# decadenza/SimpleStereo

Measured on AMD Instinct MI355X. Metric: disparity MPixels/s (H*W*nDisp per second), higher is better.
Workload: dtype f32

## Files before the change

### simplestereo_amd/build.py

```python
import os
import shutil
import subprocess

_PKG = os.path.dirname(os.path.abspath(__file__))
_SRC = os.path.join(_PKG, "csrc")
LIB_PATH = os.path.join(_PKG, "libssamd.so")
HIPCC_FLAGS = ["--offload-arch=gfx950", "-O3", "-std=c++17", "-shared", "-fPIC", "-fno-slp-vectorize",
               "-Wno-int-to-pointer-cast"]


def _sources():
    return sorted(os.path.join(_SRC, f) for f in os.listdir(_SRC) if f.endswith((".hip", ".h", ".inc")))


def needs_build():
    if not os.path.exists(LIB_PATH):
        return True
    t = os.path.getmtime(LIB_PATH)
    deps = _sources() + [os.path.join(os.path.dirname(_PKG), "include", "ssamd.h")]
    return any(os.path.getmtime(s) > t for s in deps if os.path.exists(s))


UNITS = [("ssamd_api.hip", []),
         ("asw_pipe_tu.hip", ["-mllvm", "--amdgpu-sched-strategy=max-memory-clause"]),
         ("asw_wave6_tu.hip", ["-mllvm", "--amdgpu-sched-strategy=max-ilp"])]


def build_native(force=False, verbose=False):
    if not force and not needs_build():
        return LIB_PATH
    hipcc = shutil.which("hipcc") or "/opt/rocm/bin/hipcc"
    if not os.path.exists(hipcc):
        raise RuntimeError("hipcc not found: libssamd.so cannot be built (ROCm toolchain required)")
    flags = [f for f in HIPCC_FLAGS if f != "-shared"]
    objs, procs = [], []
    for src, extra in UNITS:
        obj = os.path.join(_SRC, os.path.splitext(src)[0] + ".o")
        cmd = [hipcc] + flags + extra + ["-c", "-o", obj, os.path.join(_SRC, src)]
        if verbose:
            print(" ".join(cmd))
        procs.append((cmd, subprocess.Popen(cmd)))
        objs.append(obj)
    for cmd, p in procs:
        if p.wait() != 0:
            raise subprocess.CalledProcessError(p.returncode, cmd)
    cmd = [hipcc, "--offload-arch=gfx950", "-shared", "-fPIC", "-o", LIB_PATH + ".tmp"] + objs
    if verbose:
        print(" ".join(cmd))
    subprocess.check_call(cmd)
    os.replace(LIB_PATH + ".tmp", LIB_PATH)
    for o in objs:
        os.remove(o)
    return LIB_PATH


if __name__ == "__main__":
    print(build_native(force=True, verbose=True))
```

### simplestereo_amd/csrc/asw_kernels.hip.h

```cpp
#pragma once
#include "common.hip.h"

namespace ssamd {

static constexpr int ASW_RX = 8;
static constexpr int ASW_RD = 4;
static constexpr int ASW_WB = 4;
static constexpr int ASW_MAX_THREADS = 768;
__host__ __device__ constexpr int asw_nwr(int rx) { return (rx + ASW_RD - 1 + 3) / 4 * 4; }
static_assert(ASW_RD == 4 && asw_nwr(8) == 12 && asw_nwr(4) == 8, "the main loop is unrolled for 8x4 and 4x4 register tiles");

struct AswGeom {
    int Tx, XG, DG, Dc, nchunks, threads;
    int Rx;
    int nL, nR, nRc, SR, Se, emask;
    int SL, hL, hR;
    int wseg, wlen;
    int JC;
    int e2;
    int e_bytes;
    int pipe;
    int NC, JCmax;
    int dephase;
    int wave_rx;
    int off_wL, off_wR, off_e, off_labL, off_labR, off_bgrL, off_bgrR, off_bestL, off_bestR, off_cen, off_prox;
    int lds_bytes;
    int lds_bytes_evol;
};

struct AswExactQueue {
    u64 *entries;
    uint32_t *ekeys;
    unsigned int *counter;
    unsigned char *flagL, *flagR;
    unsigned char *zeroL, *zeroR;
    unsigned char *zrow;
    unsigned int W;
    unsigned int cap;
    uint32_t tol;
    float sat_abs;
    uint32_t deep;
};

struct AswArgs {
    const PixRec *recL, *recR;
    const float *prox;
    u64 *keyL;
    u64 *keyR;
    int16_t *disp;
    const unsigned char *evol;
    int erow0, erows, evolW;
    float *costs;
    int cost_keys;
    int H, W, win, pad, minD, maxD, row0, rows;
    int ystep;
    int yb0;
    int yskip_at, yskip;
    float kC;
    AswExactQueue xq;
    AswGeom g;
};

struct AswPipeTileId { int win, XG, DG, JC; };
__host__ __device__ constexpr int asw_cx_round_up(int v, int m) { return (v + m - 1) / m * m; }
__host__ __device__ constexpr int asw_cx_max(int a, int b) { return a > b ? a : b; }
__host__ __device__ constexpr AswGeom asw_pipe_geom_constexpr(AswPipeTileId t)
{
    AswGeom g{};
    const int win = t.win, p = win / 2;
    g.Rx = 8; g.JC = t.JC; g.pipe = 1; g.wave_rx = 0; g.e2 = 1; g.nchunks = 1;
    g.NC = (win + t.JC / 2) / t.JC;
    g.JCmax = asw_cx_max(t.JC, win - (g.NC - 1) * t.JC);
    g.XG = t.XG; g.DG = t.DG;
    g.Tx = 8 * t.XG; g.Dc = ASW_RD * t.DG;
    g.threads = asw_cx_round_up(t.XG * t.DG, 64);
    g.dephase = g.threads / 64 >= 12 ? 1 : 0;
    g.nL = g.Tx + 2 * p;
    g.nRc = g.Tx + g.Dc - 1;
    g.nR = g.nRc + 2 * p;
    g.hL = 0; g.hR = 0;
    g.SL = asw_cx_round_up(g.Tx, 4);
    g.SR = asw_cx_round_up(g.nRc + 1, 4);
    g.Se = 16 * ((t.DG + 3) / 4);
    g.emask = 0;
    const int wrows = 2 * g.JCmax;
    int off = 0;
    g.off_wL = off; off = (off + wrows * g.SL * 4 + 15) & ~15;
    g.off_wR = off; off = (off + wrows * g.SR * 4 + 15) & ~15;
    g.e_bytes = (g.nL * g.Se + 15) & ~15;
    g.off_e = off; off = (off + g.e_bytes * 2 + 15) & ~15;
    g.off_labL = off; off = (off + g.nL * 16 * 2 + 15) & ~15;
    g.off_labR = off; off = (off + g.nR * 16 * 2 + 15) & ~15;
    g.off_bestL = off; off = (off + g.Tx * 8 + 15) & ~15;
    g.off_bestR = off; off = (off + (g.nRc + 1) * 8 + 15) & ~15;
    g.off_cen = off; off = (off + (g.Tx + g.nRc) * 16 + 15) & ~15;
    g.off_prox = off; off = (off + win * 4 * 2 + 15) & ~15;
    g.lds_bytes_evol = off;
    g.off_bgrL = off; off = (off + g.nL * 4 * 2 + 15) & ~15;
    g.off_bgrR = off; off = (off + g.nR * 4 * 2 + 15) & ~15;
    g.lds_bytes = off;
    return g;
}
template <int SLC, int SRC, int SEC> struct AswPipeTile { static constexpr AswPipeTileId id{35, 1, 1, 16}; };
template <> struct AswPipeTile<120, 316, 208> { static constexpr AswPipeTileId id{35, 15, 49, 16}; };
template <> struct AswPipeTile<88, 348, 272> { static constexpr AswPipeTileId id{35, 11, 65, 16}; };
template <> struct AswPipeTile<216, 284, 80> { static constexpr AswPipeTileId id{35, 27, 17, 16}; };
inline bool asw_pipe_geom_matches(const AswGeom &a, const AswGeom &b)
{
    return a.pipe == b.pipe && a.Rx == b.Rx && a.JC == b.JC && a.NC == b.NC && a.JCmax == b.JCmax && a.XG == b.XG && a.DG == b.DG && a.Tx == b.Tx &&
           a.Dc == b.Dc && a.threads == b.threads && a.dephase == b.dephase && a.nL == b.nL && a.nRc == b.nRc && a.nR == b.nR && a.SL == b.SL &&
           a.SR == b.SR && a.Se == b.Se && a.e_bytes == b.e_bytes && a.off_wL == b.off_wL && a.off_wR == b.off_wR && a.off_e == b.off_e &&
           a.off_labL == b.off_labL && a.off_labR == b.off_labR && a.off_bestL == b.off_bestL && a.off_bestR == b.off_bestR &&
           a.off_cen == b.off_cen && a.off_prox == b.off_prox && a.off_bgrL == b.off_bgrL && a.off_bgrR == b.off_bgrR &&
           a.lds_bytes == b.lds_bytes && a.lds_bytes_evol == b.lds_bytes_evol && a.e2 == b.e2;
// ... 574 lines not shown
```

### simplestereo_amd/csrc/asw_pipe_kernel.hip.h

```cpp
#pragma once
#include "asw_kernels.hip.h"
#ifndef SSAMD_KERNEL_TU
#include "lab_kernels.hip.h"
#endif

namespace ssamd {

#ifndef SSAMD_KERNEL_TU
static constexpr int TADV_COLS = 64;
template <bool BYTES>
__device__ __forceinline__ void asw_tad_tile(const void *__restrict__ srcL, const void *__restrict__ srcR, unsigned char *__restrict__ evol,
                                             int W, int pad, int minD, int Dc, int Se, int erow0, int erows, int evolW, int rd, long long npix_total,
                                             int bx, int by, int bz, char *smem)
{
    uint32_t *const sL = reinterpret_cast<uint32_t *>(smem);
    uint32_t *const sR = sL + TADV_COLS;
    const int r = erow0 + by, z = bz, uc0 = bx * TADV_COLS;
    const int P = Se >> 2, dlo = minD + z * Dc, dhi = dlo + Dc - 1;
    const int u0 = uc0 - pad, xr0 = u0 - dhi;
    auto pixel = [&](const void *src, int col) -> uint32_t {
        const size_t q = (size_t)r * W + col;
        if constexpr (BYTES) {
            typedef uint32_t __attribute__((aligned(1))) u32_unaligned;
            const uint8_t *const b = reinterpret_cast<const uint8_t *>(src) + 3 * q;
// ... 41 lines not shown
    }
}

__global__ __launch_bounds__(256) void asw_tad_volume_kernel(const PixRec *__restrict__ recL, const PixRec *__restrict__ recR,
                                                             unsigned char *__restrict__ evol, int W, int pad, int minD, int Dc,
                                                             int Se, int erow0, int erows, int evolW, int rd = 4)
{
    extern __shared__ __attribute__((aligned(16))) char smem[];
    asw_tad_tile<false>(recL, recR, evol, W, pad, minD, Dc, Se, erow0, erows, evolW, rd, 0, blockIdx.x, blockIdx.y, blockIdx.z, smem);
}

struct AswPrepassArgs {
    const uint8_t *bgrL, *bgrR;
    PixRec *recL, *recR;
    unsigned char *evol;
    long long npix_total;
    int W, pad, minD, Dc, Se, erow0, erows, evolW, rd;
    int lab_blocks, ex, ey;
};
__global__ __launch_bounds__(256) void asw_prepass_kernel(const AswPrepassArgs P)
{
    extern __shared__ __attribute__((aligned(16))) char smem[];
    if ((int)blockIdx.x < P.lab_blocks) {
        SSAMD_LAB_TABLES_IN_LDS(T)
        const long long np = (long long)P.erows * P.W, first = (long long)P.erow0 * P.W;
        const uint8_t *const bl = P.bgrL + 3 * first, *const br = P.bgrR + 3 * first;
        PixRec *const rl = P.recL + first, *const rr = P.recR + first;
        typedef uint32_t __attribute__((aligned(1))) u32_unaligned;
        for (long long q = (long long)blockIdx.x * blockDim.x + threadIdx.x; q < 2 * np; q += (long long)P.lab_blocks * blockDim.x) {
            const bool right = q >= np;
            const long long p = right ? q - np : q;
            const uint8_t *const bgr = right ? br : bl;
            uint32_t B, G, R;
            if (p + 1 < np) {
                const uint32_t v = *reinterpret_cast<const u32_unaligned *>(bgr + 3 * p);
                B = v & 0xff; G = (v >> 8) & 0xff; R = (v >> 16) & 0xff;
            } else {
                B = bgr[3 * p]; G = bgr[3 * p + 1]; R = bgr[3 * p + 2];
            }
            PixRec o;
            bgr_to_lab(B, G, R, o.L, o.a, o.b, T);
            o.bgrx = B | (G << 8) | (R << 16);
            (right ? rr : rl)[p] = o;
        }
        return;
    }
    const int b = (int)blockIdx.x - P.lab_blocks, bx = b % P.ex, by = (b / P.ex) % P.ey, bz = b / (P.ex * P.ey);
    asw_tad_tile<true>(P.bgrL, P.bgrR, P.evol, P.W, P.pad, P.minD, P.Dc, P.Se, P.erow0, P.erows, P.evolW, P.rd, P.npix_total, bx, by, bz, smem);
}

#endif

template <bool WITH_COSTS, int SLC = 0, int SRC = 0, int SEC = 0, bool CG = false>
__global__ __launch_bounds__(ASW_MAX_THREADS, 3) void asw_aggregate_pipe_kernel(const AswArgs A)
{
    constexpr bool STATIC = SLC > 0;
    static_assert(!CG || STATIC, "compile-time geometry belongs to a static tile");
    constexpr int RX = ASW_RX;
    constexpr int NWR = asw_nwr(RX);
    extern __shared__ __attribute__((aligned(16))) char smem[];
    constexpr AswGeom SG = asw_pipe_geom_constexpr(AswPipeTile<SLC, SRC, SEC>::id);
    static_assert(!STATIC || (SG.SL == SLC && SG.SR == SRC && SG.Se == SEC), "the strides name the tile");
    const AswGeom &g = CG ? SG : A.g;
    float *const wL = reinterpret_cast<float *>(smem + g.off_wL);
    float *const wR = reinterpret_cast<float *>(smem + g.off_wR);
    unsigned char *const eT0 = reinterpret_cast<unsigned char *>(smem + g.off_e);
    float4 *const labL = reinterpret_cast<float4 *>(smem + g.off_labL);
    float4 *const labR = reinterpret_cast<float4 *>(smem + g.off_labR);
    uint32_t *const bgrL = reinterpret_cast<uint32_t *>(smem + g.off_bgrL);
    uint32_t *const bgrR = reinterpret_cast<uint32_t *>(smem + g.off_bgrR);
    u64 *const bestL = reinterpret_cast<u64 *>(smem + g.off_bestL);
    u64 *const bestR = reinterpret_cast<u64 *>(smem + g.off_bestR);
    float4 *const cenLab = reinterpret_cast<float4 *>(smem + g.off_cen);

    const int tid = threadIdx.x, nthr = blockDim.x;
    const int W = A.W, win = CG ? AswPipeTile<SLC, SRC, SEC>::id.win : A.win, p = CG ? AswPipeTile<SLC, SRC, SEC>::id.win / 2 : A.pad;
    const int Tx = g.Tx, Dc = g.Dc, nL = g.nL, nR = g.nR, nRc = g.nRc, SR = g.SR, Se = g.Se;
    const int JC = g.JC, NC = g.NC;
    int bx = blockIdx.x;
    if ((gridDim.x & 7) == 0) bx = (bx & 7) * (gridDim.x >> 3) + (bx >> 3);
    const int x0 = bx * Tx;
    const int y = asw_out_row(A, blockIdx.y);
    const int dlo = A.minD + blockIdx.z * Dc;
    const int dhi = dlo + Dc - 1;
    if (min(x0 + Tx - 1, W - 1) - dlo < 0) {
        if (A.disp)
            for (int k = threadIdx.x; k < Tx && x0 + k < W; k += blockDim.x)
                A.disp[(size_t)(y - A.row0) * W + x0 + k] = (int16_t)(x0 + k);
        return;
    }
    const int segL_lo = x0 - p, xrc_lo = x0 - dhi, segR_lo = xrc_lo - p;
    const int phase = g.dephase ? __builtin_amdgcn_readfirstlane((int)(threadIdx.x >> 8)) : 1;

    float accN[RX][ASW_RD], accS[RX][ASW_RD];
#pragma unroll
    for (int a = 0; a < RX; ++a)
#pragma unroll
        for (int b = 0; b < ASW_RD; ++b) { accN[a][b] = 0.f; accS[a][b] = 0.f; }

    for (int k = tid; k < Tx; k += nthr) bestL[k] = KEY_NONE;
    for (int k = tid; k <= nRc; k += nthr) bestR[k] = KEY_NONE;
    for (int c = tid; c < Tx + nRc; c += nthr) {
        const bool isL = c < Tx;
        const int ccol = isL ? x0 + c : xrc_lo + (c - Tx);
        float4 v = make_float4(0.f, 0.f, 0.f, 0.f);
        if ((unsigned)ccol < (unsigned)W) {
            const PixRec q = (isL ? A.recL : A.recR)[(size_t)y * W + ccol];
            v = make_float4(q.L, q.a, q.b, 1.f);
        }
        cenLab[c] = v;
    }

    const int i_lo = max(0, p - y), i_hi = min(win, A.H + p - y);

    auto stage_row = [&](int i) {
        int tids = threadIdx.x;
        asm volatile("" : "+v"(tids));
        const int buf = i & 1, r = y - p + i;
        const PixRec *const rowL = A.recL + (size_t)r * W;
        const PixRec *const rowR = A.recR + (size_t)r * W;
        for (int k = tids; k < nL + nR; k += nthr) {
            const bool isL = k < nL;
            const int idx = isL ? k : k - nL;
            const int col = (isL ? segL_lo : segR_lo) + idx;
            PixRec v;
            v.L = __builtin_inff();
            v.a = v.b = 0.f;
            v.bgrx = 0u;
            if ((unsigned)col < (unsigned)W) v = (isL ? rowL : rowR)[col];
            (isL ? labL + buf * nL : labR + buf * nR)[idx] = make_float4(v.L, v.a, v.b, 0.f);
            if (!A.evol) (isL ? bgrL + buf * nL : bgrR + buf * nR)[idx] = v.bgrx;
        }
    };
    auto build_e = [&](int i, int t_lo, int t_hi) {
        int tidb = threadIdx.x;
        asm volatile("" : "+v"(tidb));
        unsigned char *const eT = eT0 + (i & 1) * g.e_bytes;
        const uint32_t *const bgrLc = bgrL + (i & 1) * nL, *const bgrRc = bgrR + (i & 1) * nR;
        const int e_q = nthr / nL, e_r = nthr - e_q * nL;
        int t = t_lo + tidb;
        int sp = t / nL, ul = t - sp * nL;
        while (t < t_hi) {
            const uint32_t lp = bgrLc[ul];
            const uint32_t *const rp = bgrRc + (ul + (Dc - 1) - 8 * sp);
            uint32_t lo = 0, hi = 0;
#pragma unroll
            for (int k = 0; k < 4; ++k) {
                lo |= min(__builtin_amdgcn_sad_u8(lp, rp[-k], 0u), 40u) << (8 * k);
                hi |= min(__builtin_amdgcn_sad_u8(lp, rp[-4 - k], 0u), 40u) << (8 * k);
            }
            uint32_t *const dst = reinterpret_cast<uint32_t *>(eT + ul * Se) + 2 * sp;
            dst[0] = lo;
            if (2 * sp + 1 < g.DG) dst[1] = hi;
            t += nthr; ul += e_r; sp += e_q;
            if (ul >= nL) { ul -= nL; ++sp; }
        }
    };
    auto load_e = [&](int i) {
        int tidd = threadIdx.x;
        asm volatile("" : "+v"(tidd));
        const int r = y - p + i;
        const unsigned char *const src = A.evol + (((size_t)blockIdx.z * A.erows + (r - A.erow0)) * (size_t)A.evolW + x0) * Se;
        unsigned char *const dst = eT0 + (i & 1) * g.e_bytes;
        const int bytes = nL * Se, lane16 = (tidd & 63) * 16;
        for (int k = __builtin_amdgcn_readfirstlane(tidd >> 6) * 1024; k < bytes; k += (nthr >> 6) * 1024)
            if (k + lane16 < bytes)
                __builtin_amdgcn_global_load_lds((const void *)(src + k + lane16),
                                                 (__attribute__((address_space(3))) void *)(dst + k), 16, 0, 0);
    };
    auto build_weights = [&](int i, int jb, int je, int rb) {
        static_assert(ASW_WB == 4, "the remainder below is written out for batches of four");
        typedef const __attribute__((address_space(4))) float cfloat;
        int tidw = threadIdx.x;
        asm volatile("" : "+v"(tidw));
        const int wave = __builtin_amdgcn_readfirstlane(tidw >> 6), lane = tidw & 63;
        constexpr int NTHR = STATIC ? asw_cx_round_up((SLC / ASW_RX) * ((SRC - SLC) / ASW_RD), 64) : 0;
        static_assert(!STATIC || (SG.Tx == SLC && SG.nRc == SRC - 1 && SG.threads == NTHR), "the strides name the centres and the threads");
        const int TxB = STATIC ? SLC : Tx, nRcB = STATIC ? SRC - 1 : nRc, nw = (STATIC ? NTHR : nthr) >> 6;
        const int nLw = (TxB + 63) >> 6, ncw = nLw + ((nRcB + 63) >> 6);
        const float4 *const labLc = labL + (i & 1) * nL, *const labRc = labR + (i & 1) * nR;
        cfloat *const prow = reinterpret_cast<cfloat *>(reinterpret_cast<uintptr_t>(A.prox)) + i * win;
        auto batch = [&](auto n_, const float4 &cen, const float4 *sp, cfloat *pp, float *wp, int stride) {
            constexpr int N = decltype(n_)::value;
            float4 tp[N];
            float pr[N], wv[N];
#pragma unroll
            for (int u = 0; u < N; ++u) { tp[u] = sp[u]; pr[u] = pp[u]; }
#pragma unroll
            for (int u = 0; u < N; ++u) {
                asm volatile("" ::"v"(tp[u].w));
                const float dL = tp[u].x - cen.x, da = tp[u].y - cen.y, db = tp[u].z - cen.z;
                wv[u] = fmaf(db, db, fmaf(da, da, dL * dL));
            }
#pragma unroll
            for (int u = 0; u < N; ++u) wv[u] = __builtin_amdgcn_sqrtf(wv[u]);
#pragma unroll
            for (int u = 0; u < N; ++u) wv[u] = asw_weight_finish(wv[u], A.kC, pr[u]);
#pragma unroll
            for (int u = 0; u < N; ++u) wp[u * stride] = wv[u];
        };
        auto build_side = [&](auto left_, int cc, int jb_t, int je_t) {
            constexpr bool LEFT = decltype(left_)::value;
            const int stride = LEFT ? (STATIC ? SLC : g.SL) : (STATIC ? SRC : SR);
            if (cc >= (LEFT ? TxB : nRcB)) return;
            const float4 cen = cenLab[(LEFT ? 0 : TxB) + cc];
            asm volatile("" ::"v"(cen.w));
            const float4 *sp = (LEFT ? labLc : labRc) + cc + jb_t;
            cfloat *pp = prow + jb_t;
            float *wp = (LEFT ? wL : wR) + cc + (rb + jb_t - jb) * stride;
            int j = jb_t;
#pragma nounroll
            for (; j + ASW_WB <= je_t; j += ASW_WB, sp += ASW_WB, pp += ASW_WB, wp += ASW_WB * stride)
                batch(std::integral_constant<int, ASW_WB>{}, cen, sp, pp, wp, stride);
            const int rem = je_t - j;
            if (rem == 1) batch(std::integral_constant<int, 1>{}, cen, sp, pp, wp, stride);
            else if (rem == 2) batch(std::integral_constant<int, 2>{}, cen, sp, pp, wp, stride);
            else if (rem == 3) batch(std::integral_constant<int, 3>{}, cen, sp, pp, wp, stride);
        };
        int full = 0;
        while (full + nw <= ncw) full += nw;
        const int rest = ncw - full;
        int slen = je - jb, nseg = 1;
        if (rest > 0 && full > 0) {
            int per = 0;
            for (int a = rest; a <= nw; a += rest) ++per;
            for (slen = ASW_WB; slen * per < je - jb;) slen += ASW_WB;
            while (nseg * slen < je - jb) ++nseg;
        }
        for (int t = wave; t < full + rest * nseg; t += nw) {
            int cw = t, jb_t = jb, je_t = je;
            if (t >= full && nseg > 1) {
                int q = t - full, sgm = 0;
                while (q >= rest) { q -= rest; ++sgm; }
                cw = full + q;
                jb_t = jb + sgm * slen;
                je_t = min(je, jb_t + slen);
            }
            if (cw < nLw) build_side(std::true_type{}, 64 * cw + lane, jb_t, je_t);
            else build_side(std::false_type{}, 64 * (cw - nLw) + lane, jb_t, je_t);
        }
    };
    auto chunk_end = [&](int c) { return c == NC - 1 ? win : (c + 1) * JC; };
    const int nE = nL * ((g.DG + 1) >> 1);
    auto build_next = [&](int i, int c, int cb) {
        const bool more_rows = i + 1 < i_hi;
        if (c == 0 && more_rows) stage_row(i + 1);
        if (c == 0 && more_rows && A.evol) load_e(i + 1);
        if (c + 1 < NC || more_rows) {
            const int cn = c + 1 < NC ? c + 1 : 0;
            build_weights(c + 1 < NC ? i : i + 1, cn * JC, chunk_end(cn), (cb ^ 1) * g.JCmax);
        }
        if (c >= 1 && more_rows && !A.evol) build_e(i + 1, (int)((long long)nE * (c - 1) / (NC - 1)), (int)((long long)nE * c / (NC - 1)));
    };

    stage_row(i_lo);
    if (A.evol) load_e(i_lo);
    __syncthreads();
    if (!A.evol) build_e(i_lo, 0, nE);
    build_weights(i_lo, 0, chunk_end(0), 0);

    const int DGe = max(1, min(g.DG, (min(min(x0 + Tx, W) - 1, x0 + Tx - 1) - dlo) / ASW_RD + 1));
    const int nact = g.XG * DGe;
    int pk_xd;
    bool run;
    {
        const int tidm = threadIdx.x;
        int xg, dg;
        const int F = DGe >> 4, Lo = DGe & 15, nfull = g.XG * F;
        const int grp16 = tidm >> 4, r16 = tidm & 15;
        if (grp16 < nfull) {
            xg = grp16 / F;
            int gi = grp16 - xg * F;
            if (xg & 1) gi = F - 1 - gi;
            dg = 16 * gi + r16;
        } else {
            const int q = tidm - 16 * nfull;
            xg = Lo ? q / Lo : g.XG;
            dg = 16 * F + (Lo ? q - xg * Lo : 0);
        }
        pk_xd = xg | (dg << 16);
        const bool tile_live = tidm < nact && x0 + RX * xg < W && dlo + ASW_RD * dg <= A.maxD &&
                               x0 + RX * xg + RX - 1 - (dlo + ASW_RD * dg) >= 0;
        run = __builtin_amdgcn_ballot_w64(tile_live) != 0 && tidm < nact;
    }

    int cb = 0;
#pragma nounroll
    for (int i = i_lo; i < i_hi; ++i) {
        const unsigned char *const eT = eT0 + (i & 1) * g.e_bytes;
        AswRow ew[RX];

#pragma nounroll
        for (int c = 0; c < NC; ++c) {
            __syncthreads();
            const int jc = c * JC, jend = chunk_end(c);
            const int rb = cb * g.JCmax;
            if (phase == 0) build_next(i, c, cb);
            if (run) {
                const int xg = pk_xd & 0xffff, dg = pk_xd >> 16;
                const unsigned char *erow = eT + (RX * xg + (jc == 0 ? 0 : RX - 1 + jc)) * Se + 4 * dg;
                if (jc == 0) {
#pragma unroll
                    for (int n = 0; n < RX - 1; ++n) {
                        asw_row_unpack(ew[n], *reinterpret_cast<const uint32_t *>(erow));
                        erow += Se;
                    }
                }
                const float *wlp = wL + rb * g.SL + 8 * xg;
// ... 3 lines not shown
    if (j0 + (JJ) < jend) {                                                                         \
        const uint32_t epk = *reinterpret_cast<const uint32_t *>(erow + (STATIC ? (JJ) * SEC : 0)); \
        if constexpr (!STATIC) erow += Se;                                                          \
        float wl[RX], wr[NWR];                                                                      \
        {                                                                                           \
            const float *const wl_ = wlp + (STATIC ? (JJ) * SLC : 0);                              \
            const float *const wr_ = wrp + (STATIC ? (JJ) * SRC : 0);                              \
            const float4 v0 = *reinterpret_cast<const float4 *>(wl_);                              \
            wl[0] = v0.x; wl[1] = v0.y; wl[2] = v0.z; wl[3] = v0.w;                                 \
            const float4 v1 = *reinterpret_cast<const float4 *>(wl_ + 4);                          \
            wl[4] = v1.x; wl[5] = v1.y; wl[6] = v1.z; wl[7] = v1.w;                                 \
            const float4 r0 = *reinterpret_cast<const float4 *>(wr_);                              \
            const float4 r1 = *reinterpret_cast<const float4 *>(wr_ + 4);                          \
            const float4 r2 = *reinterpret_cast<const float4 *>(wr_ + 8);                          \
            asm volatile("" ::"v"(r2.w));       \
            wr[0] = r0.x; wr[1] = r0.y; wr[2] = r0.z; wr[3] = r0.w;                                 \
            wr[4] = r1.x; wr[5] = r1.y; wr[6] = r1.z; wr[7] = r1.w;                                 \
            wr[8] = r2.x; wr[9] = r2.y; wr[10] = r2.z; wr[11] = r2.w;                               \
        }                                                                                           \
        if constexpr (!STATIC) { wlp += g.SL; wrp += SR; }                                         \
               \
        _Pragma("unroll") for (int xi = 0; xi < RX; ++xi) {                                         \
            if (xi == RX - 1) asw_row_unpack(ew[((JJ) + RX - 1) % RX], epk);                        \
            const AswRow &row_ = ew[((JJ) + xi) % RX];                                              \
            _Pragma("unroll") for (int di = 0; di < ASW_RD; ++di) {                                 \
                const float w_ = wl[xi] * wr[xi - di + ASW_RD - 1];                                 \
                accN[xi][di] = fmaf(w_, row_.e[di], accN[xi][di]);                                  \
                accS[xi][di] = fmaf(w_, row_.c[di], accS[xi][di]);                                  \
            }                                                                                       \
        }                                                                                           \
    }
                    SSAMD_PSTEP(0) SSAMD_PSTEP(1) SSAMD_PSTEP(2) SSAMD_PSTEP(3)
                    SSAMD_PSTEP(4) SSAMD_PSTEP(5) SSAMD_PSTEP(6) SSAMD_PSTEP(7)
#undef SSAMD_PSTEP
                    if constexpr (STATIC) { erow += RX * SEC; wlp += RX * SLC; wrp += RX * SRC; }
                }
            }
            if (phase != 0) build_next(i, c, cb);
            cb ^= 1;
        }
    }

    int tidf = threadIdx.x;
    asm volatile("" : "+v"(tidf));
#define ASW_EPI_RD ASW_RD
#define ASW_EPI_LIVE (tidf < nact)
#define ASW_EPI_XG(live) (pk_xd & 0xffff)
#define ASW_EPI_DG(live) (pk_xd >> 16)
#define ASW_EPI_TX Tx
#define ASW_EPI_NRC nRc
#define ASW_EPI_TID tid
#define ASW_EPI_NTHR nthr
#define ASW_EPI_SYNC() __syncthreads()
#define ASW_EPI_ROW (size_t)(y - A.row0) * W
#include "asw_epilogue.inc"
}

}
```

### simplestereo_amd/csrc/ssamd_api.hip

```cpp
#include <hip/hip_runtime.h>

#include <algorithm>
#include <array>
#include <atomic>
#include <list>
#include <map>
#include <thread>
#include <cmath>
#include <cstdarg>
#include <cstdio>
#include <cstdlib>
#include <cstring>
#include <mutex>
#include <string>
#include <vector>

#include "../../include/ssamd.h"
#include "asw_kernels.hip.h"
#include "asw_pipe_kernel.hip.h"
#include "asw_wave_kernel.hip.h"
#include "asw_wave6_kernel.hip.h"
#include "asw_alt_kernels.hip.h"
namespace ssamd {
#define SSAMD_PIPE_INSTANCE(C, SL, SR, SE) extern template __global__ void asw_aggregate_pipe_kernel<C, SL, SR, SE>(const AswArgs);
// ... 104 lines not shown
    std::vector<hipEvent_t> pool;
    double ms[SSAMD_K_COUNT] = {0};
    long long n[SSAMD_K_COUNT] = {0};
    hipEvent_t get()
    {
        if (!pool.empty()) { hipEvent_t e = pool.back(); pool.pop_back(); return e; }
        hipEvent_t e = nullptr;
        (void)hipEventCreate(&e);
        return e;
    }
    void drain()
    {
        for (auto &p : pending) {
            float t = 0.f;
            if (hipEventSynchronize(p.b) == hipSuccess && hipEventElapsedTime(&t, p.a, p.b) == hipSuccess) {
                ms[p.slot] += t;
                n[p.slot] += 1;
            }
            pool.push_back(p.a);
            pool.push_back(p.b);
        }
        pending.clear();
    }
};

struct TableEntry {
    int k0 = 0; double k1 = 0;
    DevBuf dev;
    std::vector<unsigned char> host;
};
struct TableCache {
    std::list<TableEntry> entries;
    size_t max_entries;
    explicit TableCache(size_t n) : max_entries(n) {}
    TableEntry *find(int k0, double k1)
    {
        for (auto it = entries.begin(); it != entries.end(); ++it)
            if (it->k0 == k0 && it->k1 == k1) {
                entries.splice(entries.begin(), entries, it);
                return &entries.front();
            }
        return nullptr;
    }
};

struct Ctx {
    std::mutex mu;
    int dev = -1;
    int cus = 256;
    bool lut_ready = false;
    hipStream_t stream = nullptr;
    DevBuf imgL, imgR, recL, recR, keyL, keyR, disp, costs, lab, altq, evol, altdisp;
    DevBuf xlabL, xlabR, xflags, xqueue, xcost, xslots, xctr, xraw, xwtab;
    DevBuf uwIn, uwOut;
    DevBuf ftpBand, ftpPhase;
    std::map<int, DevBuf> ftpTabs;
    int32_t *ftpBandHost = nullptr;
    size_t ftpBandHostCap = 0;
    hipEvent_t ftp_band_copied = nullptr;
    unsigned int xcap = 0, xrawcap = 0;
    TableCache proxTabs{8}, gswTabs{4}, proxTabs64{8};
    std::map<const void *, int> max_dyn_lds;
    hipEvent_t scratch_free = nullptr;
    int evol_small_calls = 0;
    long long evol_fallbacks = 0;
    long long tail_splits = 0;
    long long exact_calls = 0;
    long long static_tile_mismatch = 0;
    Profile prof;
};

Ctx g_ctx[16];

struct DeviceGuard {
    int saved = -1;
    DeviceGuard() { if (hipGetDevice(&saved) != hipSuccess) saved = -1; }
    ~DeviceGuard() { if (saved >= 0) (void)hipSetDevice(saved); }
    DeviceGuard(const DeviceGuard &) = delete;
    DeviceGuard &operator=(const DeviceGuard &) = delete;
};

int grant_dyn_lds(Ctx &c, const void *kernel, int bytes);

struct Timed {
    Ctx &c; hipStream_t s; int slot; hipEvent_t a = nullptr, b = nullptr;
    Timed(Ctx &c_, hipStream_t s_, int slot_) : c(c_), s(s_), slot(slot_)
    {
        if (c.prof.on) { a = c.prof.get(); b = c.prof.get(); (void)hipEventRecord(a, s); }
    }
    ~Timed()
    {
        if (a) { (void)hipEventRecord(b, s); c.prof.pending.push_back({a, b, slot}); }
    }
};

struct CtxLock {
    DeviceGuard guard;
    std::unique_lock<std::mutex> lk;
    Ctx *c = nullptr;
    Ctx *operator->() { return c; }
    Ctx &operator*() { return *c; }
};

int get_ctx(int device, CtxLock &out)
{
    int n = 0;
    if (hipGetDeviceCount(&n) != hipSuccess || n <= 0)
        return fail(SSAMD_ENODEVICE, "no HIP device visible: libssamd has no CPU fallback");
    if (device < 0) device = out.guard.saved >= 0 ? out.guard.saved : 0;
    if (device >= n || device >= 16) return fail(SSAMD_EINVAL, "device ordinal %d out of range (%d visible)", device, n);
    HIP_TRY(hipSetDevice(device));
    Ctx &c = g_ctx[device];
    out.lk = std::unique_lock<std::mutex>(c.mu);
    out.c = &c;
    if (c.dev < 0) {
        c.dev = device;
        int cus = 0;
        if (hipDeviceGetAttribute(&cus, hipDeviceAttributeMultiprocessorCount, device) == hipSuccess && cus > 0) c.cus = cus;
        else (void)hipGetLastError();
        HIP_TRY(hipStreamCreateWithFlags(&c.stream, hipStreamNonBlocking));
// ... 538 lines not shown
    if (r.lab_pending && tiles + r.lab_blocks < (1ll << 31)) {
        AswPrepassArgs pa;
        pa.bgrL = r.dL; pa.bgrR = r.dR; pa.recL = (PixRec *)c.recL.ptr; pa.recR = (PixRec *)c.recR.ptr;
        pa.evol = (unsigned char *)c.evol.ptr; pa.npix_total = (long long)r.H * r.W;
        pa.W = r.W; pa.pad = r.p; pa.minD = r.minD; pa.Dc = Dc; pa.Se = Se; pa.erow0 = r.r0; pa.erows = erows; pa.evolW = evolW;
        pa.rd = rd;
        pa.lab_blocks = r.lab_blocks; pa.ex = (int)egrid.x; pa.ey = (int)egrid.y;
        if (int grc = grant_dyn_lds(c, (const void *)asw_prepass_kernel, (int)elds)) return grc;
        hipLaunchKernelGGL(asw_prepass_kernel, dim3((unsigned)(tiles + r.lab_blocks)), dim3(256), elds, s, pa);
        HIP_TRY(hipGetLastError());
        r.lab_pending = false;
        return SSAMD_OK;
    }
    if (r.lab_pending) {
        r.lab_pending = false;
        if (int lrc = asw_lab_records(r)) return lrc;
    }
    if (int grc = grant_dyn_lds(c, (const void *)asw_tad_volume_kernel, (int)elds)) return grc;
    hipLaunchKernelGGL(asw_tad_volume_kernel, egrid, dim3(256), elds, s, (const PixRec *)c.recL.ptr, (const PixRec *)c.recR.ptr,
                       (unsigned char *)c.evol.ptr, r.W, r.p, r.minD, Dc, Se, r.r0, erows, evolW, rd);
    HIP_TRY(hipGetLastError());
    return SSAMD_OK;
}

template <class Args> void asw_fill_args(Args &x, const AswRun &r, const AswGeom &g)
{
    const bool direct = asw_is_direct(r, g);
    x.recL = (const PixRec *)r.c.recL.ptr; x.recR = (const PixRec *)r.c.recR.ptr;
    x.prox = r.d_prox;
    x.keyL = direct ? nullptr : (u64 *)r.c.keyL.ptr;
    x.keyR = r.consistent ? (u64 *)r.c.keyR.ptr : nullptr;
    x.disp = direct ? r.d_disp : nullptr;
    x.costs = r.d_costs;
    x.cost_keys = 0;
    x.xq = r.xq_kernel;
    x.evol = r.evol; x.erow0 = r.r0; x.erows = r.r1 - r.r0; x.evolW = r.evolW;
    x.H = r.H; x.W = r.W; x.win = r.win; x.pad = r.p; x.minD = r.minD; x.maxD = r.maxD; x.row0 = r.row0; x.rows = r.rows;
    x.kC = (float)(-1.4426950408889634 / r.gammaC);
    x.ystep = r.alternate ? 2 : 1;
    x.yb0 = 0;
    x.yskip_at = r.skip > 0 ? r.skip_at : 0x7fffffff; x.yskip = r.skip;
}

int asw_launch_pipe(AswRun &r, const AswArgs &a, const dim3 &grid)
{
    Ctx &c = r.c;
    const AswGeom &g = a.g;
    const AswKernel pk = asw_pick_pipe_kernel(c, g, r.win, r.d_costs != nullptr, r.t.asw_static);
    const int pipe_lds = a.evol ? g.lds_bytes_evol : g.lds_bytes;
    if (pipe_lds > 160 * 1024) return fail(SSAMD_ELIMIT, "this tile needs the TAD volume (LDS %d bytes without it)", pipe_lds);
    if (int grc = grant_dyn_lds(c, (const void *)pk, pipe_lds)) return grc;
    int rows_main = r.grows;
    AswGeom tail_g;
    if (!r.alternate && r.t.asw_tail != 0 && g.XG >= 4) {
        const int per_simd = (g.threads / 64 + 3) / 4;
        const long long resident = std::max(1, std::min(3 / std::max(1, per_simd), (160 * 1024) / std::max(1, pipe_lds)));
        const long long per_row = (long long)grid.x * g.nchunks, n = per_row * r.grows, slots = (long long)c.cus * resident;
        const long long full = n / slots, rem = n - full * slots;
        if (full >= 1 && rem > 0 && 2 * rem <= slots && (full < 32 || r.t.asw_tail > 0)) {
            const int rm = (int)(full * slots / per_row);
            if (rm >= 1 && rm < r.grows &&
                asw_layout_e(tail_g, r.po, r.win, (g.XG + 1) / 2, g.DG, 160 * 1024, g.JC, 8, true, false, true) && tail_g.pipe &&
                tail_g.Se == g.Se && tail_g.Dc == g.Dc &&
                (a.evol == nullptr || round_up(((r.W + tail_g.Tx - 1) / tail_g.Tx) * tail_g.Tx + 2 * r.p, 4) <= a.evolW)) {
                tail_g.nchunks = g.nchunks;
                rows_main = rm;
            }
        }
    }
    hipLaunchKernelGGL(pk, dim3(grid.x, rows_main, grid.z), dim3(g.threads), pipe_lds, r.s, a);
    HIP_TRY(hipGetLastError());
    if (rows_main < r.grows) {
        ++c.tail_splits;
        AswArgs t = a;
        t.g = tail_g;
        t.yb0 = rows_main;
        const AswKernel tk = asw_pick_pipe_kernel(c, tail_g, r.win, r.d_costs != nullptr, 0);
        const int tail_lds = a.evol ? tail_g.lds_bytes_evol : tail_g.lds_bytes;
        if (int grc = grant_dyn_lds(c, (const void *)tk, tail_lds)) return grc;
        hipLaunchKernelGGL(tk, dim3((r.W + tail_g.Tx - 1) / tail_g.Tx, r.grows - rows_main, tail_g.nchunks), dim3(tail_g.threads),
                           tail_lds, r.s, t);
        HIP_TRY(hipGetLastError());
    }
    return SSAMD_OK;
}

int asw_launch(AswRun &r, const AswGeom &g)
{
    r.geom = g;
    if (g.wave_rx) {
        AswWaveArgs wa;
        asw_fill_args(wa, r, g);
        wa.g = r.wave;
        const AswWaveKernel wk = asw_pick_wave_kernel(wa.g, r.d_costs != nullptr, r.t.wave_unroll != 0);
        const int lds = wa.g.wave_lds * wa.g.waves, xt = (r.W + wa.g.Txw - 1) / wa.g.Txw;
        if (int grc = grant_dyn_lds(r.c, (const void *)wk, lds)) return grc;
        hipLaunchKernelGGL(wk, dim3((xt + wa.g.waves - 1) / wa.g.waves, r.grows, 1), dim3(64 * wa.g.waves), lds, r.s, wa);
        HIP_TRY(hipGetLastError());
        return SSAMD_OK;
    }
    AswArgs a{};
    asw_fill_args(a, r, g);
    a.g = g;
    const dim3 grid((r.W + g.Tx - 1) / g.Tx, r.grows, g.nchunks);
    if (g.pipe) return asw_launch_pipe(r, a, grid);
    const bool chunked = g.JC < r.win;
    AswKernel kern = chunked ? (r.d_costs ? asw_aggregate_kernel<true, true> : asw_aggregate_kernel<false, true>)
                             : (r.d_costs ? asw_aggregate_kernel<true, false> : asw_aggregate_kernel<false, false>);
    if (g.Rx == 4)
        kern = chunked ? (r.d_costs ? asw_aggregate_kernel<true, true, 4> : asw_aggregate_kernel<false, true, 4>)
                       : (r.d_costs ? asw_aggregate_kernel<true, false, 4> : asw_aggregate_kernel<false, false, 4>);
    if (int grc = grant_dyn_lds(r.c, (const void *)kern, g.lds_bytes)) return grc;
    hipLaunchKernelGGL(kern, grid, dim3(g.threads), g.lds_bytes, r.s, a);
    HIP_TRY(hipGetLastError());
    return SSAMD_OK;
}

int asw_autotune(AswRun &r)
{
    hipStream_t s = r.s;
    hipEvent_t e0 = nullptr, e1 = nullptr;
    HIP_TRY(hipEventCreate(&e0));
    HIP_TRY(hipEventCreate(&e1));
// ... 398 lines not shown
}

extern "C" {

int ssamd_abi_version(void) { return SSAMD_ABI_VERSION; }
const char *ssamd_last_error(void) { return g_err.c_str(); }

int ssamd_device_count(void)
{
    int n = 0;
    if (hipGetDeviceCount(&n) != hipSuccess) return 0;
    return n;
}

const char *ssamd_kernel_name(int slot)
{
    static const char *names[SSAMD_K_COUNT] = {"asw pre-pass (asw_prepass_kernel: Lab records + TAD volume; or bgr2lab_records_pair_kernel, asw_tad_volume_kernel)", "asw aggregation kernel (asw_aggregate_pipe / _wave / asw_aggregate_kernel)",
                                               "asw finalize (wta_decode / lr_check_fill)",
                                               "gsw_aggregate_kernel", "gsw finalize (lr_check_fill)", "remap_bgr_kernel", "reproject_kernel",
                                               "asw_alt_fill_kernel", "asw fp64 tie-break pass (bgr2lab_f64_pair + asw_exact_winners / _eval / _resolve / _patch kernels)",
                                               "iir_unwrap_kernel", "ftp_phase_kernel", "np_unwrap_row_kernel / np_unwrap_col_kernel"};
    return (slot >= 0 && slot < SSAMD_K_COUNT) ? names[slot] : "";
}

int ssamd_set_option(const char *name, const char *value)
{
    if (!name) return fail(SSAMD_EINVAL, "option name is NULL");
    std::lock_guard<std::mutex> lk(g_tune_mutex);
    if (value) {
        if (!tuning_assign(g_tuning, name, value)) return fail(SSAMD_EINVAL, "unknown option %s", name);
    } else {
        const auto it = g_tuning_env.find(name);
        if (!tuning_assign(g_tuning, name, it == g_tuning_env.end() ? nullptr : it->second.c_str()))
            return fail(SSAMD_EINVAL, "unknown option %s", name);
    }
    if (std::string(name) == "SSAMD_AUTOTUNE")
        g_autotune.store(g_tuning.autotune_env != -2 ? g_tuning.autotune_env : -1);
    g_tune_version.fetch_add(1, std::memory_order_release);
    return SSAMD_OK;
}

int ssamd_counter(int device, const char *name, long long *value)
{
    if (!name || !value) return fail(SSAMD_EINVAL, "name / value is NULL");
    CtxLock c;
    int rc = get_ctx(device, c);
    if (rc) return rc;
    const std::string n(name);
    if (n == "evol_fallbacks") *value = c->evol_fallbacks;
    else if (n == "evol_bytes") *value = (long long)c->evol.cap;
    else if (n == "tail_splits") *value = c->tail_splits;
    else if (n == "exact_calls") *value = c->exact_calls;
    else if (n == "static_tile_mismatch") *value = c->static_tile_mismatch;
    else if (n == "exact_entries" || n == "exact_flagged_left" || n == "exact_flagged_right" || n == "exact_overflow" || n == "exact_raw_entries") {
        unsigned int ctr[5] = {0, 0, 0, 0, 0};
        if (c->xflags.ptr && c->exact_calls > 0) {
            HIP_TRY(hipDeviceSynchronize());
            HIP_TRY(hipMemcpy(ctr, c->xflags.ptr, sizeof(ctr), hipMemcpyDeviceToHost));
        }
        *value = n == "exact_entries" ? ctr[0] : n == "exact_flagged_left" ? ctr[1] : n == "exact_flagged_right" ? ctr[2] :
                 n == "exact_raw_entries" ? ctr[4] : ((ctr[0] > c->xcap || (c->xrawcap && ctr[4] > c->xrawcap)) ? 1 : 0);
    }
    else return fail(SSAMD_EINVAL, "unknown counter %s", name);
    return SSAMD_OK;
}

int ssamd_autotune(int on)
{
    return g_autotune.exchange(on > 0 ? 1 : (on < 0 ? -1 : 0));
}

int ssamd_asw_geometry(int width, int rows, int winSize, int maxDisparity, int minDisparity, int *out)
{
    int nD, rc = check_geometry_query(width, winSize, maxDisparity, minDisparity, out, &nD);
    if (rc) return rc;
    const Tuning &t = tune();
    const PlanOptions po{t, false};
    AswGeom g;
    if ((rc = asw_choose_geometry(g, po, width, rows, winSize, nD))) return rc;
    out[0] = g.Tx; out[1] = g.Dc; out[2] = g.nchunks; out[3] = g.threads; out[4] = g.lds_bytes;
    out[5] = (width + g.Tx - 1) / g.Tx; out[6] = rows; out[7] = g.nchunks;
    AswWaveGeom wg;
    if (g.wave_rx && asw_wave_layout(wg, po, winSize, nD, g.wave_rx, t.wave_unroll != 0)) {
        out[0] = wg.Txw * wg.waves; out[1] = wg.Dc; out[2] = 1; out[3] = 64 * wg.waves; out[4] = wg.wave_lds * wg.waves;
        out[5] = (width + out[0] - 1) / out[0]; out[7] = 1;
    }
    return SSAMD_OK;
}

int ssamd_asw_kernel_form(int width, int rows, int winSize, int maxDisparity, int minDisparity, int *out)
{
    int nD, rc = check_geometry_query(width, winSize, maxDisparity, minDisparity, out, &nD);
    if (rc) return rc;
    const Tuning &t = tune();
    AswGeom g;
    if ((rc = asw_choose_geometry(g, PlanOptions{t, false}, width, rows, winSize, nD))) return rc;
    out[0] = g.pipe; out[1] = g.Rx; out[2] = g.JC >= winSize ? 0 : g.JC; out[3] = g.pipe ? g.dephase : 0;
    out[4] = g.wave_rx & 15;
    if (g.wave_rx) { out[0] = 0; out[1] = g.wave_rx & 15; out[2] = 0; out[3] = 0; }
    return SSAMD_OK;
}

int ssamd_gsw_geometry(int width, int rows, int winSize, int maxDisparity, int minDisparity, int *out)
{
    int nD, rc = check_geometry_query(width, winSize, maxDisparity, minDisparity, out, &nD);
    if (rc) return rc;
// ... 693 lines not shown
```

### simplestereo_amd/csrc/ssamd_options.h

```cpp
#pragma once

#define SSAMD_OPTIONS(X) \
    X("SSAMD_ASW_GEOM", asw_geom, std::string, "", v, !x.empty())    \
    X("SSAMD_GSW_GEOM", gsw_geom, std::string, "", v, false) \
    X("SSAMD_ASW_PIPE", asw_pipe, int, -1, atoi(v), x >= 0)    \
    X("SSAMD_ASW_DEPHASE", asw_dephase, int, -1, atoi(v), x >= 0)    \
    X("SSAMD_ASW_EVOL", asw_evol, int, 1, atoi(v), x != 1)    \
    X("SSAMD_ASW_WAVE", asw_wave, int, -1, atoi(v) != 0 ? 1 : 0, x >= 0)    \
    X("SSAMD_ASW_WAVE_RX", wave_rx, int, 0, atoi(v), x != 0)    \
    X("SSAMD_ASW_WAVE_WG", wave_wg, int, 0, std::max(1, std::min(4, atoi(v))), x != 0)    \
    X("SSAMD_ASW_WAVE_UNROLL", wave_unroll, int, 1, atoi(v), false)    \
    X("SSAMD_ASW_WAVE_MERGE", wave_merge, int, 1, atoi(v), x != 1)    \
    X("SSAMD_ASW_STATIC", asw_static, int, 1, atoi(v), x != 1)    \
    X("SSAMD_ASW_EVOL_MAX_MB", evol_max_mb, int, 0, std::max(0, atoi(v)), x != 0)    \
    X("SSAMD_ASW_WAVE_RD", wave_rd, int, 0, atoi(v), x != 0)    \
    X("SSAMD_ASW_NO_E2", no_e2, bool, false, true, x) \
    X("SSAMD_ASW_XOR_ONLY", xor_only, bool, false, true, x) \
    X("SSAMD_MULTI_ALLOW_REPEAT", multi_allow_repeat, bool, false, true, false) \
    X("SSAMD_ALT_QUEUE_CAP", alt_queue_cap, int, 0, std::max(1, atoi(v)), false)    \
    X("SSAMD_AUTOTUNE", autotune_env, int, -2, atoi(v) > 0 ? 1 : (atoi(v) < 0 ? -1 : 0), false)    \
    X("SSAMD_ASW_EVOL_FAIL", evol_fail, int, 0, atoi(v), false)    \
    X("SSAMD_ASW_TAIL", asw_tail, int, -1, atoi(v), false)    \
    X("SSAMD_ASW_WAVE_CREG", wave_creg, int, 1, atoi(v), x != 1)    \
    X("SSAMD_ASW_LDS_RELAX", lds_relax, int, 1, atoi(v), x != 1)    \
    X("SSAMD_ASW_PREPASS_FUSE", prepass_fuse, int, 1, atoi(v), false)    \
    X("SSAMD_EXACT_TOL", exact_tol, int, 128, std::max(0, atoi(v)), false)    \
    X("SSAMD_EXACT_CAP", exact_cap, int, 0, std::max(1, atoi(v)), false)    \
    X("SSAMD_EXACT_RAWCAP", exact_rawcap, int, 0, std::max(1, atoi(v)), false)    \
    X("SSAMD_UNWRAP_ROWS", unwrap_rows, int, 0, std::max(0, std::min(UNWRAP_MAX_ROWS, atoi(v))), false)

struct Tuning {
#define X(NAME, MEMBER, TYPE, UNSET, PARSE, FORCES) TYPE MEMBER = UNSET;
    SSAMD_OPTIONS(X)
#undef X
};

bool tuning_assign(Tuning &t, const std::string &name, const char *v)
{
#define X(NAME, MEMBER, TYPE, UNSET, PARSE, FORCES) \
    if (name == NAME) { if (v) t.MEMBER = PARSE; else t.MEMBER = UNSET; return true; }
    SSAMD_OPTIONS(X)
#undef X
    return false;
}

const char *const kTuningNames[] = {
#define X(NAME, MEMBER, TYPE, UNSET, PARSE, FORCES) NAME,
    SSAMD_OPTIONS(X)
#undef X
};

bool asw_geometry_forced(const Tuning &t)
{
#define X(NAME, MEMBER, TYPE, UNSET, PARSE, FORCES) { const TYPE &x = t.MEMBER; (void)x; if (FORCES) return true; }
    SSAMD_OPTIONS(X)
#undef X
    return false;
}
```

Baseline: 10750.

## Add persistent-worker scheduling with per-XCC atomic work queues to ASW pipe kernel

Wraps the pipe aggregation kernel body in a per-item lambda and, when there are many tiles, launches only as many blocks as fit resident on the device. Those blocks pull tile indices from eight atomic ticket queues chosen by XCC id, stealing from other queues once their own is empty. The next ticket is prefetched during row staging to hide the atomic latency. This aims to cut block launch and tail overhead and keep each XCC's caches local. In exchange it adds atomics, extra barriers, a completion counter and a compiler flag that disables machine LICM.

```diff
diff --git a/simplestereo_amd/build.py b/simplestereo_amd/build.py
--- a/simplestereo_amd/build.py
+++ b/simplestereo_amd/build.py
@@ -22,7 +22,7 @@
 
 
 UNITS = [("ssamd_api.hip", []),
-         ("asw_pipe_tu.hip", ["-mllvm", "--amdgpu-sched-strategy=max-memory-clause"]),
+         ("asw_pipe_tu.hip", ["-mllvm", "--amdgpu-sched-strategy=max-memory-clause", "-mllvm", "-disable-machine-licm"]),
          ("asw_wave6_tu.hip", ["-mllvm", "--amdgpu-sched-strategy=max-ilp"])]
 
 
diff --git a/simplestereo_amd/csrc/asw_kernels.hip.h b/simplestereo_amd/csrc/asw_kernels.hip.h
--- a/simplestereo_amd/csrc/asw_kernels.hip.h
+++ b/simplestereo_amd/csrc/asw_kernels.hip.h
@@ -59,7 +59,11 @@
     float kC;
     AswExactQueue xq;
     AswGeom g;
+    unsigned int *pq;
+    int pq_nx, pq_ny, pq_items;
 };
+static constexpr int ASW_PQ_QUEUES = 8;
+static constexpr int ASW_PQ_LINE = 32;
 
 struct AswPipeTileId { int win, XG, DG, JC; };
 __host__ __device__ constexpr int asw_cx_round_up(int v, int m) { return (v + m - 1) / m * m; }
diff --git a/simplestereo_amd/csrc/asw_pipe_kernel.hip.h b/simplestereo_amd/csrc/asw_pipe_kernel.hip.h
--- a/simplestereo_amd/csrc/asw_pipe_kernel.hip.h
+++ b/simplestereo_amd/csrc/asw_pipe_kernel.hip.h
@@ -117,7 +117,7 @@
 #endif
 
 template <bool WITH_COSTS, int SLC = 0, int SRC = 0, int SEC = 0, bool CG = false>
-__global__ __launch_bounds__(ASW_MAX_THREADS, 3) void asw_aggregate_pipe_kernel(const AswArgs A)
+__global__ __launch_bounds__(ASW_MAX_THREADS, 3) void asw_aggregate_pipe_kernel(const AswArgs A0)
 {
     constexpr bool STATIC = SLC > 0;
     static_assert(!CG || STATIC, "compile-time geometry belongs to a static tile");
@@ -126,6 +126,10 @@
     extern __shared__ __attribute__((aligned(16))) char smem[];
     constexpr AswGeom SG = asw_pipe_geom_constexpr(AswPipeTile<SLC, SRC, SEC>::id);
     static_assert(!STATIC || (SG.SL == SLC && SG.SR == SRC && SG.Se == SEC), "the strides name the tile");
+    uint32_t *const pq_next = reinterpret_cast<uint32_t *>(smem + (CG ? SG : A0.g).off_prox);
+    int pq_q = 0;
+    auto run_item = [&](const AswArgs &A, const int ibx, const int iby, const int ibz, const int inx) __attribute__((always_inline)) {
+    const bool persist = A.pq != nullptr;
     const AswGeom &g = CG ? SG : A.g;
     float *const wL = reinterpret_cast<float *>(smem + g.off_wL);
     float *const wR = reinterpret_cast<float *>(smem + g.off_wR);
@@ -142,18 +146,26 @@
     const int W = A.W, win = CG ? AswPipeTile<SLC, SRC, SEC>::id.win : A.win, p = CG ? AswPipeTile<SLC, SRC, SEC>::id.win / 2 : A.pad;
     const int Tx = g.Tx, Dc = g.Dc, nL = g.nL, nR = g.nR, nRc = g.nRc, SR = g.SR, Se = g.Se;
     const int JC = g.JC, NC = g.NC;
-    int bx = blockIdx.x;
-    if ((gridDim.x & 7) == 0) bx = (bx & 7) * (gridDim.x >> 3) + (bx >> 3);
+    size_t Wz = (size_t)W;
+    asm volatile("" : "+s"(Wz));
+    int bx = ibx;
+    if ((inx & 7) == 0) bx = (bx & 7) * (inx >> 3) + (bx >> 3);
     const int x0 = bx * Tx;
-    const int y = asw_out_row(A, blockIdx.y);
-    const int dlo = A.minD + blockIdx.z * Dc;
+    const int y = asw_out_row(A, iby);
+    const int dlo = A.minD + ibz * Dc;
     const int dhi = dlo + Dc - 1;
     if (min(x0 + Tx - 1, W - 1) - dlo < 0) {
         if (A.disp)
             for (int k = threadIdx.x; k < Tx && x0 + k < W; k += blockDim.x)
-                A.disp[(size_t)(y - A.row0) * W + x0 + k] = (int16_t)(x0 + k);
+                A.disp[(size_t)(y - A.row0) * Wz + x0 + k] = (int16_t)(x0 + k);
+        if (persist) {
+            if (threadIdx.x == 0) *pq_next = atomicAdd(A.pq + pq_q * ASW_PQ_LINE, 1u);
+            __syncthreads();
+        }
         return;
     }
+    uint32_t pq_ticket = 0;
+    if (persist && threadIdx.x == 0) pq_ticket = atomicAdd(A.pq + pq_q * ASW_PQ_LINE, 1u);
     const int segL_lo = x0 - p, xrc_lo = x0 - dhi, segR_lo = xrc_lo - p;
     const int phase = g.dephase ? __builtin_amdgcn_readfirstlane((int)(threadIdx.x >> 8)) : 1;
 
@@ -170,7 +182,7 @@
         const int ccol = isL ? x0 + c : xrc_lo + (c - Tx);
         float4 v = make_float4(0.f, 0.f, 0.f, 0.f);
         if ((unsigned)ccol < (unsigned)W) {
-            const PixRec q = (isL ? A.recL : A.recR)[(size_t)y * W + ccol];
+            const PixRec q = (isL ? A.recL : A.recR)[(size_t)y * Wz + ccol];
             v = make_float4(q.L, q.a, q.b, 1.f);
         }
         cenLab[c] = v;
@@ -182,8 +194,8 @@
         int tids = threadIdx.x;
         asm volatile("" : "+v"(tids));
         const int buf = i & 1, r = y - p + i;
-        const PixRec *const rowL = A.recL + (size_t)r * W;
-        const PixRec *const rowR = A.recR + (size_t)r * W;
+        const PixRec *const rowL = A.recL + (size_t)r * Wz;
+        const PixRec *const rowR = A.recR + (size_t)r * Wz;
         for (int k = tids; k < nL + nR; k += nthr) {
             const bool isL = k < nL;
             const int idx = isL ? k : k - nL;
@@ -225,7 +237,7 @@
         int tidd = threadIdx.x;
         asm volatile("" : "+v"(tidd));
         const int r = y - p + i;
-        const unsigned char *const src = A.evol + (((size_t)blockIdx.z * A.erows + (r - A.erow0)) * (size_t)A.evolW + x0) * Se;
+        const unsigned char *const src = A.evol + (((size_t)ibz * A.erows + (r - A.erow0)) * (size_t)A.evolW + x0) * Se;
         unsigned char *const dst = eT0 + (i & 1) * g.e_bytes;
         const int bytes = nL * Se, lane16 = (tidd & 63) * 16;
         for (int k = __builtin_amdgcn_readfirstlane(tidd >> 6) * 1024; k < bytes; k += (nthr >> 6) * 1024)
@@ -319,6 +331,7 @@
     };
 
     stage_row(i_lo);
+    if (persist && threadIdx.x == 0) *pq_next = pq_ticket;
     if (A.evol) load_e(i_lo);
     __syncthreads();
     if (!A.evol) build_e(i_lo, 0, nE);
@@ -428,8 +441,46 @@
 #define ASW_EPI_TID tid
 #define ASW_EPI_NTHR nthr
 #define ASW_EPI_SYNC() __syncthreads()
-#define ASW_EPI_ROW (size_t)(y - A.row0) * W
+#define ASW_EPI_ROW (size_t)(y - A.row0) * Wz
 #include "asw_epilogue.inc"
+    };
+
+    int dead = 0;
+    if (A0.pq) {
+        uint32_t xcc;
+        asm volatile("s_getreg_b32 %0, hwreg(HW_REG_XCC_ID)" : "=s"(xcc));
+        pq_q = (int)(xcc & (ASW_PQ_QUEUES - 1));
+        if (threadIdx.x == 0) *pq_next = atomicAdd(A0.pq + pq_q * ASW_PQ_LINE, 1u);
+        __syncthreads();
+    }
+    for (;;) {
+        typedef const __attribute__((address_space(4))) AswArgs *KernArgs;
+        uintptr_t ka = reinterpret_cast<uintptr_t>(__builtin_amdgcn_kernarg_segment_ptr());
+        asm volatile("" : "+s"(ka));
+        const AswArgs &A = *(const AswArgs *)reinterpret_cast<KernArgs>(ka);
+        const bool persist = A.pq != nullptr;
+        int ibx = blockIdx.x, iby = blockIdx.y, ibz = blockIdx.z, inx = gridDim.x;
+        if (persist) {
+            int item = pq_q + ASW_PQ_QUEUES * __builtin_amdgcn_readfirstlane((int)*pq_next);
+            while ((unsigned)item >= (unsigned)A.pq_items) {
+                if (++dead == ASW_PQ_QUEUES) return;
+                pq_q = (pq_q + 1) & (ASW_PQ_QUEUES - 1);
+                __syncthreads();
+                if (threadIdx.x == 0) *pq_next = atomicAdd(A.pq + pq_q * ASW_PQ_LINE, 1u);
+                __syncthreads();
+                item = pq_q + ASW_PQ_QUEUES * __builtin_amdgcn_readfirstlane((int)*pq_next);
+            }
+            __syncthreads();
+            inx = A.pq_nx;
+            const int row = item / inx;
+            ibx = item - row * inx;
+            ibz = row / A.pq_ny;
+            iby = row - ibz * A.pq_ny;
+        }
+        run_item(A, ibx, iby, ibz, inx);
+        if (!persist) return;
+        if (threadIdx.x == 0) atomicAdd(reinterpret_cast<unsigned long long *>(A.pq + ASW_PQ_QUEUES * ASW_PQ_LINE), 1ull);
+    }
 }
 
 }
diff --git a/simplestereo_amd/csrc/ssamd_api.hip b/simplestereo_amd/csrc/ssamd_api.hip
--- a/simplestereo_amd/csrc/ssamd_api.hip
+++ b/simplestereo_amd/csrc/ssamd_api.hip
@@ -180,6 +180,7 @@
     hipStream_t stream = nullptr;
     DevBuf imgL, imgR, recL, recR, keyL, keyR, disp, costs, lab, altq, evol, altdisp;
     DevBuf xlabL, xlabR, xflags, xqueue, xcost, xslots, xctr, xraw, xwtab;
+    DevBuf pq;
     DevBuf uwIn, uwOut;
     DevBuf ftpBand, ftpPhase;
     std::map<int, DevBuf> ftpTabs;
@@ -194,6 +195,7 @@
     long long evol_fallbacks = 0;
     long long tail_splits = 0;
     long long exact_calls = 0;
+    long long persist_launches = 0;
     long long static_tile_mismatch = 0;
     Profile prof;
 };
@@ -838,10 +840,11 @@
     if (int grc = grant_dyn_lds(c, (const void *)pk, pipe_lds)) return grc;
     int rows_main = r.grows;
     AswGeom tail_g;
+    const int per_simd = (g.threads / 64 + 3) / 4;
+    const long long resident = std::max(1, std::min(3 / std::max(1, per_simd), (160 * 1024) / std::max(1, pipe_lds)));
+    const long long per_row = (long long)grid.x * g.nchunks, slots = (long long)c.cus * resident;
     if (!r.alternate && r.t.asw_tail != 0 && g.XG >= 4) {
-        const int per_simd = (g.threads / 64 + 3) / 4;
-        const long long resident = std::max(1, std::min(3 / std::max(1, per_simd), (160 * 1024) / std::max(1, pipe_lds)));
-        const long long per_row = (long long)grid.x * g.nchunks, n = per_row * r.grows, slots = (long long)c.cus * resident;
+        const long long n = per_row * r.grows;
         const long long full = n / slots, rem = n - full * slots;
         if (full >= 1 && rem > 0 && 2 * rem <= slots && (full < 32 || r.t.asw_tail > 0)) {
             const int rm = (int)(full * slots / per_row);
@@ -854,7 +857,24 @@
             }
         }
     }
-    hipLaunchKernelGGL(pk, dim3(grid.x, rows_main, grid.z), dim3(g.threads), pipe_lds, r.s, a);
+    const long long items = per_row * rows_main;
+    long long workers = r.t.asw_persist > 0 ? std::min<long long>(r.t.asw_persist, slots) : (r.t.asw_persist < 0 && items >= 64 * slots ? slots : 0);
+    workers = std::min(workers, items);
+    if (workers > 0 && items < (1ll << 30)) {
+        const size_t pq_bytes = (size_t)(ASW_PQ_QUEUES + 1) * ASW_PQ_LINE * 4;
+        if (!c.pq.ptr) {
+            if (int prc = c.pq.reserve(pq_bytes)) return prc;
+            HIP_TRY(hipMemsetAsync(c.pq.ptr, 0, pq_bytes, r.s));
+        }
+        HIP_TRY(hipMemsetAsync(c.pq.ptr, 0, (size_t)ASW_PQ_QUEUES * ASW_PQ_LINE * 4, r.s));
+        AswArgs pa = a;
+        pa.pq = (unsigned int *)c.pq.ptr;
+        pa.pq_nx = (int)grid.x; pa.pq_ny = rows_main; pa.pq_items = (int)items;
+        ++c.persist_launches;
+        hipLaunchKernelGGL(pk, dim3((unsigned)workers), dim3(g.threads), pipe_lds, r.s, pa);
+    } else {
+        hipLaunchKernelGGL(pk, dim3(grid.x, rows_main, grid.z), dim3(g.threads), pipe_lds, r.s, a);
+    }
     HIP_TRY(hipGetLastError());
     if (rows_main < r.grows) {
         ++c.tail_splits;
@@ -1359,6 +1379,15 @@
     else if (n == "tail_splits") *value = c->tail_splits;
     else if (n == "exact_calls") *value = c->exact_calls;
     else if (n == "static_tile_mismatch") *value = c->static_tile_mismatch;
+    else if (n == "pipe_persist_launches") *value = c->persist_launches;
+    else if (n == "pipe_persist_items") {
+        unsigned long long done = 0;
+        if (c->pq.ptr) {
+            HIP_TRY(hipDeviceSynchronize());
+            HIP_TRY(hipMemcpy(&done, (const unsigned int *)c->pq.ptr + ASW_PQ_QUEUES * ASW_PQ_LINE, sizeof(done), hipMemcpyDeviceToHost));
+        }
+        *value = (long long)done;
+    }
     else if (n == "exact_entries" || n == "exact_flagged_left" || n == "exact_flagged_right" || n == "exact_overflow" || n == "exact_raw_entries") {
         unsigned int ctr[5] = {0, 0, 0, 0, 0};
         if (c->xflags.ptr && c->exact_calls > 0) {
diff --git a/simplestereo_amd/csrc/ssamd_options.h b/simplestereo_amd/csrc/ssamd_options.h
--- a/simplestereo_amd/csrc/ssamd_options.h
+++ b/simplestereo_amd/csrc/ssamd_options.h
@@ -21,6 +21,7 @@
     X("SSAMD_AUTOTUNE", autotune_env, int, -2, atoi(v) > 0 ? 1 : (atoi(v) < 0 ? -1 : 0), false)    \
     X("SSAMD_ASW_EVOL_FAIL", evol_fail, int, 0, atoi(v), false)    \
     X("SSAMD_ASW_TAIL", asw_tail, int, -1, atoi(v), false)    \
+    X("SSAMD_ASW_PERSIST", asw_persist, int, -1, atoi(v), x > 0)    \
     X("SSAMD_ASW_WAVE_CREG", wave_creg, int, 1, atoi(v), x != 1)    \
     X("SSAMD_ASW_LDS_RELAX", lds_relax, int, 1, atoi(v), x != 1)    \
     X("SSAMD_ASW_PREPASS_FUSE", prepass_fuse, int, 1, atoi(v), false)    \
```

Measured after the change: 10980 (median of 6 runs). 2.1% higher.
